# mengyao/Complete-Striped-Smith-Waterman-Library

Hardware: AMD Instinct MI355X
Metric: GCUPS (higher is better)
Workload: dtype int16x2 (packed; reference u8/int16 semantics); 1 GPU; BASELINE config 2: 100k x 150 bp reads vs 1 Mb target; 2/-2/3/1, score_size 2, flag 0; reads_per_gpu=100000, read_len=150, ref_len=1000000

## Files before the change

### complete-striped-smith-waterman-library_amd/csrc/lanes.h

```cpp
#ifndef SSW_LANES_H
#define SSW_LANES_H

#include <stdint.h>

typedef uint32_t u32;
typedef short s16x2 __attribute__((ext_vector_type(2)));
typedef unsigned short u16x2 __attribute__((ext_vector_type(2)));
typedef uint32_t u32x4 __attribute__((ext_vector_type(4)));
typedef uint32_t u32x2 __attribute__((ext_vector_type(2)));

#ifdef SSW_SIMT_EMU
#include "simt_emu.h"
#else
#include <hip/hip_runtime.h>
#define SSW_DEV __device__ __forceinline__
#define SSW_DEVM __device__ __forceinline__
#define SSW_HD __host__ __device__ inline
#define SSW_DYN_LDS(name) extern __shared__ __attribute__((aligned(16))) unsigned char name[]

SSW_DEV u32 xl_row_shr1_zero(u32 v) { return (u32)__builtin_amdgcn_mov_dpp((int)v, 0x111, 0xf, 0xf, true); }
SSW_DEV u32 xl_row_shr1_keep(u32 keep, u32 v) { return (u32)__builtin_amdgcn_update_dpp((int)keep, (int)v, 0x111, 0xf, 0xf, false); }
SSW_DEV u32 xl_row_shr1_umax(u32 v, u32 b)
{
	u32 r;
// ... 117 lines not shown
#define FR_DEAD 32768
SSW_DEV u32 fr_pack(int lo, int hi) { return (u32)lo + ((u32)hi << 16); }
SSW_DEV bool fr_borrows(u32 s0) { return (int32_t)s0 < 0 && s0 != fr_pack(FR_DEAD, FR_DEAD); }
template <bool HPAIR> SSW_DEV void fr_add_pair(u32 h0, u32 h1, u32 s0, u32 s1, u32& x0, u32& x1)
{
	unsigned long long h = (unsigned long long)h1 << 32 | h0, s = (unsigned long long)s1 << 32 | s0;
#ifdef SSW_SIMT_EMU
	if ((((unsigned long long)h0 + s0) >> 32 != 0) != fr_borrows(s0)) emu::fail("fr_add_pair: the low word's carry does not match its borrow");
#else
	asm("" : "+v"(s));
	if constexpr (HPAIR) asm("" : "+v"(h));
#endif
	const unsigned long long x = h + s;
	x0 = (u32)x; x1 = (u32)(x >> 32);
}
SSW_DEV u32 umax32(u32 a, u32 b) { return a > b ? a : b; }
#ifdef SSW_SIMT_EMU
SSW_DEV u32 pk_gt_mask(u32 a, u32 b) { return ((a & 0xffffu) > (b & 0xffffu) ? 0xffffu : 0u) | ((a >> 16) > (b >> 16) ? 0xffff0000u : 0u); }
#else
SSW_DEV u32 pk_gt_mask(u32 a, u32 b)
{
	u32 r;
	asm("v_pk_sub_u16 %0, %1, %2 clamp\n\tv_pk_min_u16 %0, %0, %3\n\tv_pk_mul_lo_u16 %0, %0, %4" : "=&v"(r) : "v"(a), "v"(b), "v"(0x00010001u), "v"(0xffffffffu));
	return r;
}
#endif
SSW_DEV u32 pk_addw(u32 a, u32 b) { return __builtin_bit_cast(u32, (u16x2)(__builtin_bit_cast(u16x2, a) + __builtin_bit_cast(u16x2, b))); }
SSW_DEV int fr_phi(int step, int lane, int GL, int base, int kmask, int gapE) { return base + ((step & kmask) + GL - lane) * gapE; }
SSW_DEV u32 pk_dup(int v) { return ((u32)v & 0xffffu) * 0x10001u; }
SSW_DEV u32 pk_make(int lo, int hi) { return ((u32)lo & 0xffffu) | ((u32)hi << 16); }
// ... 43 lines not shown
```

### complete-striped-smith-waterman-library_amd/csrc/ssw_dev.h

```cpp
#ifndef SSW_DEV_H
#define SSW_DEV_H

#include <stdint.h>
#include <stddef.h>

#ifdef __cplusplus
extern "C" {
#endif

#define SSW_RMAX 24
#define SSW_R8MAX 23
#define SSW_MAX_N 32
#define SSW_MAX_N_WIDE 128
#define SSW_LDS_LIMIT (160 * 1024)

typedef struct {
	int32_t qa;
	int32_t qb;
} ssw_pair;

typedef struct {
	int32_t score1, score2;
	int32_t ref_begin1, ref_end1, read_begin1, read_end1, ref_end2;
	int32_t cigarLen;
// ... 32 lines not shown
	const int8_t* mat;
	int32_t n;
	uint32_t gapO2, gapE2;
	int32_t tile;
	int32_t halo;
	int32_t ntiles;
	int32_t bpp;
	uint32_t* cm16;
	uint32_t* cm8;
	int64_t cm_stride;
	uint32_t* sg16;
	uint32_t* sg8;
	int64_t seg_stride;
	int32_t form;
	int32_t fr_base, fr_kmask;
} ssw_fill_args;

typedef struct {
	const ssw_fill_args* sub;
	const int32_t* first_wg;
	const int32_t* subR;
	int32_t nsub;
} ssw_fillm_args;

struct ssw_out_rec {
	uint16_t score1, score2;
	int32_t ref_begin1, ref_end1, read_begin1, read_end1, ref_end2, cigarLen, edit_distance;
	int64_t cigar_off;
	uint16_t flag, status;
};
// ... 454 lines not shown
```

### complete-striped-smith-waterman-library_amd/csrc/ssw_host.c

```c
#include <stdlib.h>
#include <stdio.h>
#include <string.h>
#include <pthread.h>
#include "ssw.h"
#include "ssw_gpu.h"
#ifdef SSW_GPU_TEST_HOOKS
#include "ssw_gpu_diag.h"
#endif
#include "ssw_dev.h"

_Static_assert(sizeof(struct ssw_out_rec) == sizeof(ssw_gpu_result), "device record layout must equal ssw_gpu_result");
_Static_assert(sizeof(struct ssw_mate_rec) == sizeof(ssw_gpu_mates) && sizeof(ssw_gpu_mates) == 32, "device selection layout must equal ssw_gpu_mates");
_Static_assert(sizeof(struct ssw_rescue_slot) == sizeof(ssw_gpu_rescued) && sizeof(ssw_gpu_rescued) == 24, "device rescue slot layout must equal ssw_gpu_rescued");
_Static_assert(SSW_MATES_GROUP_MAX == SSW_GPU_MATES_GROUP_MAX, "the kernel's group limit is the header's");
_Static_assert(SSW_MATES_FR == SSW_GPU_MATES_FR && SSW_MATES_RF == SSW_GPU_MATES_RF && SSW_MATES_FF == SSW_GPU_MATES_FF, "the kernel's orientations are the header's");
_Static_assert(sizeof(struct ssw_best_rec) == sizeof(ssw_gpu_best) && sizeof(ssw_gpu_best) == 16, "device record layout must equal ssw_gpu_best");

struct _profile {
	const int8_t* read;
	const int8_t* mat;
	int32_t readLen;
	int32_t n;
	int8_t score_size;
};
// ... 14 lines not shown
	int overlap;
	int no_track;
	int no_seg_reduce;
	int window_int16;
	int trace_wave;
	int trace_no_lds;
	int trace_waves;
	int trace_unblocked;
	int trace_many;
	int trace_early;
	int trace_w1max, trace_w4max, trace_headroom;
	int pipe_any_count;
	int pipe_low_prio;
	int pipe_parts;
	int no_fill_half;
	int no_pipe;
	int no_lit_spec;
	int trace_no_cls80;
	int trace_diag;
	int serial_buckets;
	int no_dbx;
	int no_tail;
	int no_band;
	int call_trace;
	int db_tsub, dbx_slab;
} ssw_knobs;

#define SSW_TSTREAMS 6
#define SSW_PSTREAMS 7
#define DB_STREAMS 4
// ... 21 lines not shown
	int budget_shrunk;
	ssw_knobs kn;
	int dev_cus, dev_wave_slots;
	int device_share;
	int queue_used;
	void* hits_d[2]; void* hits_h[2]; size_t hits_cap;
};

struct ssw_gpu_seqs {
	ssw_gpu_ctx* ctx;
	int8_t* d_codes;
	int64_t* d_off;
	int64_t* h_off;
	int32_t count;
	int64_t total;
};

static __thread char g_open_err[512];

#define CALL_TRACE(what) do { if (c->kn.call_trace) fprintf(stderr, "[ssw_gpu call] %9.3f ms  %s\n", dbg_ms(), what); } while (0)

#ifdef SSW_GPU_TEST_HOOKS
static int env_int(const char* name, int dflt) { const char* e = getenv(name); return e && e[0] ? atoi(e) : dflt; }
#endif
static int env_is(const char* name, char ch) { const char* e = getenv(name); return e && e[0] == ch; }
static void knobs_load(ssw_knobs* k)
{
	memset(k, 0, sizeof *k);
	k->debug = getenv("SSW_GPU_DEBUG") != 0;
	k->call_trace = env_is("SSW_GPU_CALL_TRACE", '1');
// ... 17 lines not shown
	k->no_seg_reduce = env_is("SSW_GPU_SEG_REDUCE", '0');
	k->window_int16 = getenv("SSW_GPU_WINDOW_INT16") != 0;
	k->trace_wave = getenv("SSW_GPU_TRACE_WAVE") ? env_is("SSW_GPU_TRACE_WAVE", '1') : -1;
	k->trace_no_lds = env_is("SSW_GPU_TRACE_LDS", '0');
	{ const int v = env_int("SSW_GPU_TRACE_WAVES", 0); k->trace_waves = v == 1 || v == 4 || v == 16 ? v : 0; }
	k->trace_unblocked = env_is("SSW_GPU_TRACE_BLOCKED", '0');
	k->trace_diag = env_is("SSW_GPU_TRACE_DIAG", '1');
	if (getenv("SSW_GPU_TRACE_MANY")) k->trace_many = env_int("SSW_GPU_TRACE_MANY", 4096);
	k->serial_buckets = env_is("SSW_GPU_SERIAL_BUCKETS", '1');
	k->no_dbx = env_is("SSW_GPU_NO_DBX", '1');
	k->no_band = env_is("SSW_GPU_NO_BAND", '1');
	k->trace_no_cls80 = env_is("SSW_GPU_TRACE_CLS80", '0');
	k->no_lit_spec = env_is("SSW_GPU_LIT_SPEC", '0');
	k->no_pipe = env_is("SSW_GPU_PIPE", '0');
	k->no_fill_half = env_is("SSW_GPU_FILL_HALF", '0');
	k->pipe_low_prio = env_is("SSW_GPU_PIPE_PRIO", 'l');
	k->pipe_any_count = env_is("SSW_GPU_PIPE_EVEN", '0');
	{ const int v = env_int("SSW_GPU_TRACE_W1MAX", 0); if (v >= 2 && v <= 254) k->trace_w1max = v; }
	{ const int v = env_int("SSW_GPU_TRACE_W4MAX", 0); if (v >= 2 && v <= 3070) k->trace_w4max = v; }
	{ const int v = env_int("SSW_GPU_TRACE_HEADROOM", 0); if (v >= 2 && v <= 64) k->trace_headroom = v; }
	{ const int v = env_int("SSW_GPU_PIPE_PARTS", 0); k->pipe_parts = v >= 2 && v <= 8 ? v : 0; }
	k->trace_early = env_int("SSW_GPU_TRACE_EARLY", 0);
	k->no_tail = env_is("SSW_GPU_NO_TAIL", '1');
	{ const int v = env_int("SSW_GPU_DB_TSUB", 0); k->db_tsub = v > 0 ? v : 0; }
	{ const int v = env_int("SSW_GPU_DBX_SLAB", 0); k->dbx_slab = v > 0 ? v : 0; }
#endif
}
#ifdef SSW_GPU_TEST_HOOKS
int ssw_gpu_has_test_hooks(void) { return 1; }
#endif
// ... 173 lines not shown
	return s;
}

ssw_gpu_seqs* ssw_gpu_seqs_upload(ssw_gpu_ctx* c, const int8_t* codes, const int64_t* offsets, int32_t count)
{
	if (!c || count < 0 || !offsets || (!codes && offsets[count] != offsets[0])) { fail(c, "seqs_upload: bad arguments%s", ""); return 0; }
	ssw_shim_set_device(c->device);
	ssw_gpu_seqs* s = seqs_new(c, offsets, count);
	if (!s) return 0;
	void* const us = upload_stream(c);
	if (ssw_shim_h2d(s->d_codes, codes + offsets[0], (size_t)s->total, us) ||
	    ssw_shim_h2d(s->d_off, s->h_off, sizeof(int64_t) * ((size_t)count + 1), us) ||
	    ssw_shim_stream_sync(us)) {
		fail(c, "upload failed: %s", ssw_shim_last_error()); ssw_gpu_seqs_free(s); return 0;
	}
	return s;
}

void ssw_gpu_seqs_free(ssw_gpu_seqs* s)
{
	if (!s) return;
	if (s->ctx) ssw_shim_set_device(s->ctx->device);
	ssw_shim_free(s->d_codes); ssw_shim_free(s->d_off); free(s->h_off); free(s);
}

ssw_gpu_seqs* ssw_gpu_seqs_upload_ascii(ssw_gpu_ctx* c, const char* text, const int64_t* offsets, int32_t count, const int8_t* table128)
{
	if (!c || count < 0 || !offsets || !table128 || (!text && offsets[count] != offsets[0])) { fail(c, "seqs_upload_ascii: bad arguments%s", ""); return 0; }
	ssw_shim_set_device(c->device);
	ssw_gpu_seqs* s = seqs_new(c, offsets, count);
	if (!s) return 0;
	void* const us = upload_stream(c);
	uint8_t* d_text = (uint8_t*)ssw_shim_malloc((size_t)s->total + 64);
	int8_t* d_tab = (int8_t*)ssw_shim_malloc(128);
	int ok = d_text && d_tab;
	if (ok) {
		ssw_prep_args pa; memset(&pa, 0, sizeof pa);
		pa.text = d_text; pa.table = d_tab; pa.off = s->d_off; pa.count = count; pa.total = s->total; pa.out = s->d_codes; pa.mode = 0;
		ok = !(ssw_shim_h2d(d_text, text + offsets[0], (size_t)s->total, us) || ssw_shim_h2d(d_tab, table128, 128, us) ||
		       ssw_shim_h2d(s->d_off, s->h_off, sizeof(int64_t) * ((size_t)count + 1), us) ||
		       ssw_shim_launch_prep(&pa, us) || ssw_shim_stream_sync(us));
	}
	ssw_shim_free(d_text); ssw_shim_free(d_tab);
	if (!ok) { fail(c, "ascii upload failed: %s", ssw_shim_last_error()); ssw_gpu_seqs_free(s); return 0; }
	return s;
}

ssw_gpu_seqs* ssw_gpu_seqs_revcomp(ssw_gpu_ctx* c, const ssw_gpu_seqs* in)
{
	if (!c || !in || in->ctx != c) { fail(c, "seqs_revcomp: bad arguments%s", ""); return 0; }
	ssw_shim_set_device(c->device);
	ssw_gpu_seqs* s = seqs_new(c, in->h_off, in->count);
	if (!s) return 0;
	void* const us = upload_stream(c);
	ssw_prep_args pa; memset(&pa, 0, sizeof pa);
	pa.codes_in = in->d_codes; pa.off = in->d_off; pa.count = in->count; pa.total = in->total; pa.out = s->d_codes; pa.mode = 1;
	if (ssw_shim_h2d(s->d_off, s->h_off, sizeof(int64_t) * ((size_t)in->count + 1), us) ||
	    ssw_shim_launch_prep(&pa, us) || ssw_shim_stream_sync(us)) {
		fail(c, "revcomp failed: %s", ssw_shim_last_error()); ssw_gpu_seqs_free(s); return 0;
	}
	return s;
}

ssw_gpu_seqs* ssw_gpu_seqs_with_revcomp(ssw_gpu_ctx* c, const ssw_gpu_seqs* in)
{
	if (!c || !in || in->ctx != c || in->count > 0x3fffffff) { fail(c, "seqs_with_revcomp: bad arguments%s", ""); return 0; }
	ssw_shim_set_device(c->device);
	const int32_t n = in->count;
	int64_t* off2 = (int64_t*)malloc(sizeof(int64_t) * (2 * (size_t)n + 1));
	if (!off2) { fail(c, "out of host memory%s", ""); return 0; }
	for (int32_t i = 0; i <= n; ++i) { off2[i] = in->h_off[i]; off2[n + i] = in->total + in->h_off[i]; }
	ssw_gpu_seqs* s = seqs_new(c, off2, 2 * n);
	free(off2);
	if (!s) return 0;
	void* const us = upload_stream(c);
	ssw_prep_args pa; memset(&pa, 0, sizeof pa);
	pa.codes_in = in->d_codes; pa.off = in->d_off; pa.count = n; pa.total = in->total; pa.out = s->d_codes; pa.mode = 2;
	if (ssw_shim_h2d(s->d_off, s->h_off, sizeof(int64_t) * (2 * (size_t)n + 1), us) ||
	    ssw_shim_launch_prep(&pa, us) || ssw_shim_stream_sync(us)) {
		fail(c, "revcomp failed: %s", ssw_shim_last_error()); ssw_gpu_seqs_free(s); return 0;
	}
	return s;
}

int ssw_gpu_seqs_download(ssw_gpu_ctx* c, const ssw_gpu_seqs* s, int8_t* codes_out)
{
	if (!c || !s || !codes_out) return -1;
	ssw_shim_set_device(c->device);
	if (ssw_shim_d2h(codes_out, s->d_codes, (size_t)s->total, c->stream) || ssw_shim_stream_sync(c->stream)) return fail(c, "download failed: %s", ssw_shim_last_error());
	return 0;
}

int32_t ssw_gpu_seqs_count(const ssw_gpu_seqs* s) { return s ? s->count : 0; }

int ssw_gpu_last_timing_sized(const ssw_gpu_ctx* c, void* out, size_t out_size)
{
// ... 5 lines not shown
int ssw_gpu_last_timing(const ssw_gpu_ctx* c, ssw_gpu_timing* out) { return ssw_gpu_last_timing_sized(c, out, sizeof *out); }


static int ssw_frame_params(const ssw_knobs* kn, int64_t top, int gapO, int gapE, int minmat, int lanes, int32_t* base, int32_t* kmask)
{
	if (gapO <= gapE || gapE < 1) return 0;
	int K = 1024;
	if (kn->frame_k) { K = 16; while (K * 2 <= kn->frame_k && K < 1024) K <<= 1; }
	while (K > 64 && (int64_t)K * gapE > 4096) K >>= 1;
	const int b = (minmat < 0 ? -minmat : 0) + gapO + 2 * gapE + 8;
	const int up = lanes + 2 + (lanes == 8 ? 3 : 0);
	while (K > 64 && top + b + (int64_t)(K + up) * gapE >= 31744) K >>= 1;
	if (top + b + (int64_t)(K + up) * gapE >= 31744) return 0;
	*base = b; *kmask = K - 1;
	return 1;
}

static int32_t halo_for(int32_t P, int32_t maxmat, int32_t gapE)
{
	if (gapE <= 0) return 0x3fffffff;
	int64_t w = (int64_t)P + ((int64_t)P * (maxmat > 0 ? maxmat : 0) + gapE - 1) / gapE + 1;
	return w > 0x3fffffff ? 0x3fffffff : (int32_t)w;
}

static void* next_event(ssw_gpu_ctx* c)
{
	if (c->nev == c->capev) {
		int nc = c->capev ? c->capev * 2 : 64;
		void** ne = (void**)realloc(c->ev, sizeof(void*) * nc);
		if (!ne) return 0;
// ... 166 lines not shown
typedef struct { int32_t key, need, q; } tpend;
static int tpend_cmp(const void* a, const void* b)
{
	const tpend* x = (const tpend*)a; const tpend* y = (const tpend*)b;
	if (x->key != y->key) return x->key < y->key ? -1 : 1;
	return x->q < y->q ? -1 : x->q > y->q;
}
static int keyed_cmp(const void* a, const void* b)
{
	const keyed* x = (const keyed*)a; const keyed* y = (const keyed*)b;
	if (x->key != y->key) return x->key < y->key ? -1 : 1;
	if (x->sub != y->sub) return x->sub < y->sub ? -1 : 1;
	return x->q < y->q ? -1 : (x->q > y->q);
}

static double fill8_ops_per_row(int R)
{
	if (R == 9) return 6.5;
	int cm = 0, last = 1;
	for (int k = 0; k < 4 && k < R; ++k) {
		const int n = (R - 1 - k) / 4 + 1 + (k == 0);
		cm += (n - 1) / 2;
		if (k == 0) last += (n & 1) == 0;
		else { cm += 1 + ((n & 1) == 0); ++last; }
	}
	return (double)(4 * R + (R + 1) / 2 + (R - 1) / 4 + cm + last / 2) / R;
}

static void note_fill_kernel(ssw_gpu_ctx* c, int64_t cells, int64_t* best_cells, const char* name, double ops, int32_t R, int32_t strips)
{
	if (cells <= *best_cells) return;
	*best_cells = cells;
	snprintf(c->tm.fill_kernel, sizeof c->tm.fill_kernel, "%s", name);
	c->tm.fill_ops_per_row = ops; c->tm.fill_rows_per_lane = R; c->tm.fill_strips = strips;
}

static int chainq_check(ssw_gpu_ctx* c)
{
	if (!c->queue_used || !c->qerr.p) return 0;
	int32_t e = 0;
	c->queue_used = 0;
// ... 1340 lines not shown
static int32_t* bucket_cand(const ssw_gpu_ctx* c, const target_plan* tp, const bucket* B, const bplan* P)
{
	return B->use_x && !c->kn.no_track ? (int32_t*)(tp->base_cand + P->cand_off) : 0;
}

static int fill_args_for(const ssw_gpu_ctx* c, const batch_call* bc, const target_plan* tp, const bucket* B, const bplan* P, int32_t p0, int32_t np,
                         const fill_bufs* fb, int half, ssw_fill_args* fa)
{
	const ssw_gpu_params* prm = bc->prm;
	const int64_t top = (int64_t)16 * B->R * (bc->maxmat > 0 ? bc->maxmat : 0);
	fa->tgt = tp->d_tgt; fa->refLen = tp->refLen; fa->qcodes = bc->Q->d_codes; fa->qoff = bc->Q->d_off;
	fa->pairs = bc->d_pairs + B->first_pair + p0; fa->npairs = np; fa->mat = bc->d_mat; fa->n = bc->n;
	fa->gapO2 = bc->gapO2; fa->gapE2 = bc->gapE2; fa->tile = P->tile; fa->halo = P->halo; fa->ntiles = P->ntiles;
	fa->bpp = (P->ntiles + 15) / 16; fa->cm16 = fb->cm16; fa->cm8 = fb->cm8; fa->cm_stride = tp->stride;
	fa->sg16 = fb->sg16; fa->sg8 = fb->sg8; fa->seg_stride = tp->seg_stride;
	fa->form = 0; fa->fr_base = 0; fa->fr_kmask = 0;
	if (bc->fill_form != 0 && ssw_frame_params(&c->kn, top, prm->gapO, prm->gapE, bc->minmat, 16, &fa->fr_base, &fa->fr_kmask)) fa->form = 3;
	int32_t hb = 0, hk = 0;
	if (!half || B->use_x || fa->form != 3 || !ssw_frame_params(&c->kn, top, prm->gapO, prm->gapE, bc->minmat, 8, &hb, &hk)) return 0;
	fa->fr_base = hb; fa->fr_kmask = hk;
	return 1;
}

static void reduce_args_for(const ssw_gpu_ctx* c, const batch_call* bc, const target_plan* tp, const bucket* B, const bplan* P, int32_t p0, int32_t np,
                            const fill_bufs* fb, ssw_reduce_args* ra)
{
	const ssw_gpu_params* prm = bc->prm;
	ra->cm16 = fb->cm16; ra->cm8 = fb->cm8; ra->cm_stride = tp->stride; ra->refLen = tp->refLen; ra->pairs = bc->d_pairs + B->first_pair + p0; ra->npairs = np;
	ra->qoff = bc->Q->d_off; ra->maskLen = prm->maskLen; ra->bias = bc->bias; ra->score_size = prm->score_size;
	ra->flag = prm->flag; ra->filters = prm->filters; ra->res = bc->d_res; ra->cand = bucket_cand(c, tp, B, P); ra->tile = P->tile; ra->ntiles = P->ntiles;
	ra->sg16 = fb->sg16; ra->sg8 = fb->sg8; ra->seg_stride = tp->seg_stride;
}

static int fill_launch(ssw_gpu_ctx* c, batch_call* bc, const target_plan* tp, int b, int32_t p0, int32_t np, const fill_bufs* fb, void* st, int* ndefer)
{
	const bucket* B = &bc->bk[b]; const bplan* P = &tp->bp[b];
	const ssw_gpu_params* prm = bc->prm;
	const int use_x = B->use_x, conc = ndefer != 0;
	const int32_t n = bc->n, refLen = tp->refLen, tile = P->tile, halo = P->halo, ntiles = P->ntiles;
	ssw_fill_args fa;
	const int use_half = fill_args_for(c, bc, tp, B, P, p0, np, fb, B->half && !conc, &fa);
	int xform = 0;
	if (use_x) {
		int32_t xfr_base = 0, xfr_kmask = 0;
		if (bc->fill_form != 0 && B->lanes == 64 &&
		    ssw_frame_params(&c->kn, (int64_t)B->P16 * (bc->maxmat > 0 ? bc->maxmat : 0), prm->gapO, prm->gapE, bc->minmat, 64, &xfr_base, &xfr_kmask)) xform = 3;
		ssw_chainx_args xa; memset(&xa, 0, sizeof xa);
		xa.tgt = tp->d_tgt; xa.refLen = refLen; xa.qcodes = bc->Q->d_codes; xa.qoff = bc->Q->d_off; xa.mat = bc->d_mat; xa.n = n;
		xa.gapO2 = bc->gapO2; xa.gapE2 = bc->gapE2; xa.gapE = prm->gapE; xa.maxmat = bc->maxmat; xa.njobs = np * ntiles;
		xa.pairs = fa.pairs; xa.tile = tile; xa.halo = halo; xa.ntiles = ntiles; xa.cm16 = fb->cm16; xa.cm8 = fb->cm8;
		xa.cm_stride = tp->stride; xa.bnd = (uint32_t*)(tp->base_bnd + P->bnd_off); xa.bnd_stride = P->maxcols; xa.cand = bucket_cand(c, tp, B, P); xa.lanes = B->lanes;
		xa.sg16 = fb->sg16; xa.sg8 = fb->sg8; xa.seg_stride = tp->seg_stride;
		if (B->lanes == 64) {
			const int qgrid = chainq_grid(c, B->R, 0, n);
			if (conc ? chainq_setup(c, &xa, B->strips, (int64_t)np * ntiles, qgrid, tp->base_q + P->q_off, tp->base_cs + P->cs_off, st)
			         : chainq_prepare(c, &xa, B->strips, (int64_t)np * ntiles, qgrid)) return -1;
// ... 8 lines not shown
	if (conc) {
		fill_defer* d = &bc->defer[(*ndefer)++];
		d->fa = fa; d->R = B->R; d->wgs = (int64_t)np * fa.bpp; d->group = ssw_shim_fill_class(B->R) * 2 + (fa.form == 3);
	} else
	if (use_half ? ssw_shim_launch_fill8(B->half, &fa, st) : ssw_shim_launch_fill(B->R, &fa, st)) return fail(c, "fill launch failed: %s", ssw_shim_last_error());

	int64_t cols = 0;
	for (int32_t k = 0; k < ntiles; ++k) {
		int64_t lo = (int64_t)k * tile, hi = lo + tile < refLen ? lo + tile : refLen;
		int64_t cf = lo - halo > 0 ? lo - halo : 0;
		cols += hi - cf;
	}
	const int64_t lc = cols * (int64_t)(use_half ? 8 * B->half : B->lanes * (B->tailR ? B->R * (B->strips - 1) + B->tailR : B->R * B->strips)) * 2 * np;
	c->tm.fill_cells += lc;
	char nm[48];
	if (use_half) snprintf(nm, sizeof nm, "k_fill8<%d,frame>", B->half);
	else if (!use_x) snprintf(nm, sizeof nm, "k_fill<%d,%s>", B->R, fa.form == 3 ? "frame" : "int16");
	else if (B->lanes == 64 && B->tailR) snprintf(nm, sizeof nm, "k_chainq<%d,%s> x %d strips + 1 of %d", B->R, xform == 3 ? "frame" : "int16", B->strips - 1, B->tailR);
	else if (B->lanes == 64) snprintf(nm, sizeof nm, "k_chainq<%d,%s> x %d strips", B->R, xform == 3 ? "frame" : "int16", B->strips);
	else snprintf(nm, sizeof nm, "k_chainx<%d,16 lanes> x %d strips", B->R, B->strips);
	note_fill_kernel(c, lc, &bc->best_fill_cells, nm, use_half ? fill8_ops_per_row(B->half) : !use_x ? (fa.form == 3 ? 6.5 : 9.0) : (B->lanes == 64 && xform == 3 ? 6.5 : 9.0), use_half ? B->half : B->R, B->strips);
	return 0;
}

static int fill_bucket_series(ssw_gpu_ctx* c, batch_call* bc, const target_plan* tp, int b)
{
	const bucket* B = &bc->bk[b]; const bplan* P = &tp->bp[b];
	const int dbl = P->dbl;
	const int pipe = P->pipe;
	const fill_bufs A = bucket_bufs(tp, P);
	fill_bufs B2 = A;
	if (dbl) { B2.cm16 = (uint32_t*)tp->base_cmB16; B2.cm8 = (uint32_t*)tp->base_cmB8; }
	void *pe0 = 0, *pe1 = 0;
	if (pipe) {
		pe0 = next_event(c); pe1 = next_event(c);
		if (ssw_shim_event_record(pe0, c->stream)) return fail(c, "stream wait failed: %s", ssw_shim_last_error());
// ... 1138 lines not shown
		free(q2); free(gidx); free(gbeg); free(goff); free(tmp);
		q2 = (int32_t*)malloc(sizeof(int32_t) * 2 * (size_t)m); t2 = q2 ? q2 + m : 0;
		gidx = (int32_t*)malloc(sizeof(int32_t) * (size_t)nd); gbeg = (int64_t*)malloc(sizeof(int64_t) * (size_t)nd);
		goff = (int64_t*)malloc(sizeof(int64_t) * ((size_t)nd + 1)); tmp = (ssw_gpu_result*)malloc(sizeof(ssw_gpu_result) * (size_t)m);
		if (!q2 || !gidx || !gbeg || !goff || !tmp) { fail(c, "out of host memory%s", ""); goto out; }
		int64_t d = -1;
		goff[0] = 0;
		for (int64_t k = k0; k < k1; ++k) {
			if (k == k0 || wk[k].t != wk[k - 1].t || wk[k].b != wk[k - 1].b || wk[k].l != wk[k - 1].l) {
				++d; gidx[d] = wk[k].t; gbeg[d] = wk[k].b; goff[d + 1] = goff[d] + wk[k].l;
			}
			q2[k - k0] = qidx[wk[k].i]; t2[k - k0] = (int32_t)d;
		}
		ssw_gpu_seqs* G = seqs_new(c, goff, (int32_t)nd);
		if (!G) goto out;
		unsigned char* d_g = (unsigned char*)ssw_shim_malloc(12 * (size_t)nd);
		ssw_seqgather_args ga; memset(&ga, 0, sizeof ga);
		ga.src = T->d_codes; ga.src_off = T->d_off; ga.src_beg = (const int64_t*)d_g; ga.idx = (const int32_t*)(d_g + 8 * (size_t)nd);
		ga.dst_off = G->d_off; ga.dst = G->d_codes; ga.count = (int32_t)nd;
		const int ok = d_g && !ssw_shim_h2d((void*)ga.src_beg, gbeg, 8 * (size_t)nd, c->stream) && !ssw_shim_h2d((void*)ga.idx, gidx, 4 * (size_t)nd, c->stream) &&
		               !ssw_shim_h2d(G->d_off, G->h_off, sizeof(int64_t) * ((size_t)nd + 1), c->stream) &&
		               !ssw_shim_launch_seqgather(&ga, c->stream) && !ssw_shim_stream_sync(c->stream);
		ssw_shim_free(d_g);
		if (!ok) { fail(c, "align_windows: window gather failed: %s", ssw_shim_last_error()); ssw_gpu_seqs_free(G); goto out; }
		uint32_t* pool = 0; int64_t words = 0;
		if (align_pairs_locked(c, Q, G, q2, t2, m, prm, tmp, &pool, &words)) { ssw_gpu_seqs_free(G); goto out; }
		ssw_gpu_seqs_free(G);
		timing_add(acc, &c->tm);
		acc->t.win_copied += sum;
		if (stage_append_batch(c, st, pool, words, tmp, m, &wk[k0].i, sizeof(wkey), results)) goto out;
// ... 821 lines not shown
```

### complete-striped-smith-waterman-library_amd/csrc/ssw_kernels.hip

```cpp
#include "lanes.h"
#include "ssw_dev.h"

#define DEAD2 0x80008000u

SSW_DEV int vm_query(const ssw_vmap& m, int v) { return m.vq ? m.vq[v] : v; }
SSW_DEV const int8_t* vm_target(const ssw_vmap& m, const int8_t* tgt, int v) { return m.vq ? m.tcodes + (m.win ? m.win[m.vt[v]].start : m.toff[m.vt[v]]) : tgt; }

#define RING_BYTES 160
#define CHAIN_BYTES (RING_BYTES + 256 + 256)

template <int R> struct ChainGeom {
	static constexpr int C = (R + 3) / 4;
	static constexpr int PSTRIDE = C * 256;
	static constexpr int A8 = 16 * R - 8;
	static constexpr int TAP = A8 / R;
	static constexpr int K8 = A8 % R;
};

template <int R, int PM = 0>
SSW_DEV void build_profile(unsigned char* lds, u32 base, int first, int nthreads,
                           const int8_t* mat, int n,
                           const int8_t* qa, int lena, int reva,
                           const int8_t* qb, int lenb, int p16a = 0x7fffffff, int p16b = 0x7fffffff, int gapE = 0)
{
// ... 252 lines not shown
template <int... I> struct RowSeq {};
template <int N, int... I> struct RowSeqTo : RowSeqTo<N - 1, N - 1, I...> {};
template <int... I> struct RowSeqTo<0, I...> { typedef RowSeq<I...> type; };
template <int R, int... I> SSW_DEV void rows_set(Rows8<R>& a, u32 v, RowSeq<I...>) { ((row_at<I>(a) = v), ...); }
template <int R, int... I> SSW_DEV void rows_sub(Rows8<R>& a, u32 k, RowSeq<I...>) { ((row_at<I>(a) -= k), ...); }

template <int R> struct RowFrame8 {
	static constexpr int P = R == 9 ? 1 : 4;
	static constexpr int cls(int r) { return r % P; }
	static constexpr int KL = cls(R - 1);
	static constexpr int count(int k) { return k < R && k < P ? (R - 1 - k) / P + 1 + (k == 0) : 0; }
	static constexpr bool LEFT0 = (count(0) & 1) == 0;
	static constexpr int ROW0 = (R - 1) / P * P;
	static constexpr bool PAIR = P != 1;
	static constexpr bool HPAIR = R <= 7;
};
template <int R, int... I> SSW_DEV void rows_set_cls(Rows8<R>& a, u32 v, u32 g, RowSeq<I...>) { ((row_at<I>(a) = v + (u32)RowFrame8<R>::cls(I) * g), ...); }
SSW_DEV u32 pk_max_all(u32 a) { return a; }
SSW_DEV u32 pk_max_all(u32 a, u32 b) { return pk_max(a, b); }
template <typename... T> SSW_DEV u32 pk_max_all(u32 a, u32 b, u32 c, T... rest) { return pk_max_all(pk_max3_fr(a, b, c), rest...); }

template <int R, int r>
SSW_DEV void chain_row8(const u32x4* sc, Rows8<R>& H, Rows8<R>& E, u32& x, u32& x2, u32& f, u32& a0, u32& a1, u32& a2, u32& a3,
                        u32 c1, u32 gapE2, u32 fl0, u32 fl1, u32 fl2, u32 fl3)
{
	typedef RowFrame8<R> F;
	constexpr int P = F::P, k = F::cls(r), j = r / P + (k == 0), n = F::count(k);
	u32& Hr = row_at<r>(H); u32& Er = row_at<r>(E);
	u32& a = k == 0 ? a0 : k == 1 ? a1 : k == 2 ? a2 : a3;
	u32 xn = 0u;
	if constexpr (F::PAIR && (r & 1) == 0) xn = x2;
	else if constexpr (F::PAIR && r + 2 < R) fr_add_pair<F::HPAIR>(Hr, row_at<(r + 2 < R ? r + 1 : 0)>(H), sc[(r + 1) >> 2][(r + 1) & 3], sc[(r + 1) >> 2][(r + 2) & 3], xn, x2);
	else if constexpr (r + 1 < R) xn = Hr + sc[(r + 1) >> 2][(r + 1) & 3];
	const u32 h = pk_max3_fr(x, Er, f);
	const u32 t = h - c1;
	Er = pk_max3_fr(Er, t, k == 0 ? fl0 : k == 1 ? fl1 : k == 2 ? fl2 : fl3);
	f = pk_max(f, t);
	if (r != R - 1 && F::cls(r + 1) == 0) f -= (u32)(k + 1) * gapE2;
	if (j == 0) a = h;
	else if ((j & 1) == 0) a = pk_max3_fr(a, row_at<(r >= P ? r - P : 0)>(H), h);
	else if (j == n - 1 && k != 0) a = pk_max(a, h);
	Hr = h;
	x = xn;
}
template <int R>
SSW_DEV u32 cm_finish8(Rows8<R>& H, u32 a0, u32 a1, u32 a2, u32 a3, u32 gapE2)
{
	typedef RowFrame8<R> F;
	if constexpr (F::P == 1) {
		if constexpr (F::LEFT0) return pk_max_all(a0, row_at<F::ROW0>(H));
		else return a0;
	} else if constexpr (R >= 4) {
		const u32 b1 = a1 - gapE2, b2 = a2 - 2u * gapE2, b3 = a3 - 3u * gapE2;
		if constexpr (F::LEFT0) return pk_max_all(a0, row_at<F::ROW0>(H), b1, b2, b3);
		else return pk_max_all(a0, b1, b2, b3);
	} else if constexpr (R == 3) return pk_max_all(a0, row_at<0>(H), a1 - gapE2, a2 - 2u * gapE2);
	else if constexpr (R == 2) return pk_max_all(a0, row_at<0>(H), a1 - gapE2);
	else return pk_max_all(a0, row_at<0>(H));
}
template <int R, int... I>
SSW_DEV u32 chain_rows_fr8(const u32x4* sc, Rows8<R>& H, Rows8<R>& E, u32 d, u32& f, u32 cm, u32 c1, u32 gapE2,
                           u32 fl0, u32 fl1, u32 fl2, u32 fl3, RowSeq<I...>)
{
	u32 x, x2 = 0, a0 = cm, a1 = 0, a2 = 0, a3 = 0;
	if constexpr (RowFrame8<R>::PAIR && R >= 2) fr_add_pair<RowFrame8<R>::HPAIR>(d, row_at<0>(H), sc[0][0], sc[0][1], x, x2);
	else x = d + sc[0][0];
	(chain_row8<R, I>(sc, H, E, x, x2, f, a0, a1, a2, a3, c1, gapE2, fl0, fl1, fl2, fl3), ...);
	return cm_finish8<R>(H, a0, a1, a2, a3, gapE2);
}

template <int R>
SSW_DEV void build_profile8(unsigned char* lds, int first, int nthreads, const int8_t* mat, int n,
                            const int8_t* const (&q)[4], const int (&len)[4], bool live1, int gapE)
{
	constexpr int C = ChainGeom<R>::C;
	const int total = (n + 1) * C * 64;
	for (int w = first; w < total; w += nthreads) {
		const int b = w / (C * 64), rem = w - b * (C * 64);
		const int c = rem >> 6, l = (rem & 63) >> 2, k = rem & 3;
		const int ch = l >> 3, r = c * 4 + k, row = (l & 7) * R + r;
		u32 v;
		if (b == n || (ch && !live1)) v = fr_pack(FR_DEAD, FR_DEAD);
// ... 63 lines not shown
		if (live1) { o16[cm_stride + tc] = i16[1]; o8[cm_stride + tc] = i8[1]; }
	}
	if (gq) {
		u32 m[4];
#pragma unroll
		for (int k = 0; k < 4; ++k) m[k] = in ? (k & 1 ? i8[k >> 1] : i16[k >> 1]) : 0u;
		const u32 x16 = pk_max(xl_dpp_banks<0x128, 0xc>(m[0], m[2]), xl_dpp_banks<0x128, 0x3>(m[2], m[0]));
		const u32 x8 = pk_max(xl_dpp_banks<0x128, 0xc>(m[1], m[3]), xl_dpp_banks<0x128, 0x3>(m[3], m[1]));
		u32 y = pk_max(xl_dpp_banks<0x114, 0xa>(x16, x8), xl_dpp_banks<0x104, 0x5>(x8, x16));
		y = pk_max(y, xl_dpp_banks<DPP_QUAD_SWAP1, 0xf>(y, y));
		y = pk_max(y, xl_dpp_banks<DPP_QUAD_SWAP2, 0xf>(y, y));
		if ((l16 & 3) == 0 && (live1 || l16 < 8) && base >= store_from && base < ncols) gq[base >> 4] = y;
	}
}

template <int R>
SSW_DEV void fill_body8(const ssw_fill_args& a, const int bid, unsigned char* lds)
{
	typedef ChainGeom<R> G;
	constexpr int C = G::C;
	const int tid = (int)threadIdx.x, l16 = tid & 15, grp = tid >> 4, ch = l16 & 1, pos = l16 >> 1;
	const int pg = bid / a.bpp, tchunk = bid - pg * a.bpp;
	const bool live1 = 2 * pg + 1 < a.npairs;
	const int gapEi = (int)(a.gapE2 & 0xffffu), gapOi = (int)(a.gapO2 & 0xffffu);
	const u32 prof_bytes = (u32)(a.n + 1) * G::PSTRIDE;
	const u32 ring = prof_bytes + (u32)grp * CHAIN8_BYTES;
	const u32 rb = opaque(ring + RING_BYTES), outv = rb + 2 * PARK8_BYTES + 2 * CRING8_BYTES, carry = outv + 2 * VRING8_BYTES;
	const u32 nulloff = (u32)a.n * G::PSTRIDE;

	{
		const int8_t* q[4]; int len[4];
#pragma unroll
		for (int k = 0; k < 2; ++k) {
// ... 38 lines not shown
		if (code < 0 || code > a.n) code = a.n;
		nxt = (u32)code * G::PSTRIDE;
	}
	__syncthreads();

	const u32 zero0 = pk_dup(fr_phi(0, pos, 8, a.fr_base, a.fr_kmask, gapEi) - gapEi);
	constexpr int KL = RowFrame8<R>::KL;
	const u32 klg = (u32)KL * a.gapE2;
	u32 fl0 = zero0 + a.gapE2, fl1 = fl0 + a.gapE2, fl2 = fl1 + a.gapE2, fl3 = fl2 + a.gapE2;
	typedef typename RowSeqTo<R>::type Rows;
	Rows8<R> H, E;
	rows_set_cls(H, zero0, a.gapE2, Rows()); rows_set_cls(E, fl0, a.gapE2, Rows());
	u32 Hlast = zero0 + klg, Fout = zero0 + klg + a.gapE2, cmout = zero0, hsave = zero0 + klg;
	const u32 lane_prof = (u32)(ch * 8 + pos) * 16u;
	const u32 gO = a.gapO2 - a.gapE2, gE = a.gapE2;
	const u32 gEv = opaque(klg + gE);
	u32 fin = 0;
	const u32 park = rb + (u32)ch * PARK8_BYTES, rbl = opaque(rb + 4u * (u32)l16);
	const u32 lgd = pk_dup(l16 * gapEi);
	const bool low8 = l16 < 8;

	for (int s0 = 0; s0 < nsteps; s0 += 16) {
		if (s0 > 0 && (s0 & a.fr_kmask) == 0) {
			const u32 k = (u32)(a.fr_kmask + 1) * a.gapE2;
			rows_sub(H, k, Rows()); rows_sub(E, k, Rows());
			Hlast -= k; Fout -= k; cmout -= k; hsave -= k; fl0 -= k; fl1 -= k; fl2 -= k; fl3 -= k;
		}
		{
			const int p = (s0 + 16 + l16) & 63;
			lds_st16(lds, ring + 2u * p, nxt);
// ... 9 lines not shown
		if (s0 >= 32)
			fill_flush8(lds, rb, s0 - 32, l16, store_from, ncols, live1, o16, o8, a.cm_stride, gq, gapEi, gapOi);
		const u32 rp = ring + 2u * (u32)((s0 - pos) & 63);
#pragma unroll
		for (int j = 0; j < 16; ++j) {
			const u32 paddr = lds_ld16(lds, rp + 2u * j) + lane_prof;
			u32x4 sc[C];
#pragma unroll
			for (int c = 0; c < C; ++c) sc[c] = lds_ld128(lds, paddr + 256u * c);
			const u32 hprev = Hlast;
			const u32 hin = xl_row_shr2_umax(Hlast, KL == 0 ? fl0 : KL == 1 ? fl1 : KL == 2 ? fl2 : fl3);
			if constexpr (RowFrame8<R>::P == 1) fl0 += gE;
			else { const u32 up = fl3 + gE; fl0 = fl1; fl1 = fl2; fl2 = fl3; fl3 = up; }
			xl_row_shr2_sub_keep(fin, Fout, gEv);
			u32 f = fin, d = hsave;
			const u32 cm = chain_rows_fr8(sc, H, E, d, f, xl_row_shr2_zero(cmout), gO, gE, fl0, fl1, fl2, fl3, Rows());
			hsave = hin; Hlast = row_at<R - 1>(H); Fout = f; cmout = cm;
			if (pos == 7) {
				lds_st32(lds, park + 4u * j, cm); lds_st32(lds, park + 64u + 4u * j, f); lds_st32(lds, park + 128u + 4u * j, hprev);
			}
		}
	}
	wave_lds_fence();
	fill_stage8(lds, rbl, nsteps - 16, low8, lgd, a.fr_base, a.fr_kmask, gapEi, gE, klg);
	wave_lds_fence();
	for (int base = nsteps - 32; base < nsteps; base += 16)
		if (base >= 0) fill_flush8(lds, rb, base, l16, store_from, ncols, live1, o16, o8, a.cm_stride, gq, gapEi, gapOi);
}

template <int R>
__global__ void __launch_bounds__(256) SSW_WAVES_PER_EU(R <= 9 ? 7 : R <= 15 ? 5 : 4, 8) k_fill8(ssw_fill_args a)
{
	SSW_DYN_LDS(lds);
	fill_body8<R>(a, (int)blockIdx.x, lds);
}

template <int CLS> struct FillClass { static constexpr int LO = CLS == 0 ? 1 : CLS == 1 ? 11 : 17, HI = CLS == 0 ? 10 : CLS == 1 ? 16 : 24; };
template <int R, int CLS, int FORM> SSW_DEV void fillm_case(const ssw_fill_args& a, int bid, unsigned char* lds)
{
	if (R >= FillClass<CLS>::LO && R <= FillClass<CLS>::HI) fill_body<(R >= FillClass<CLS>::LO && R <= FillClass<CLS>::HI) ? R : FillClass<CLS>::LO, FORM>(a, bid, lds);
}
template <int CLS, int FORM>
__global__ void __launch_bounds__(256) SSW_WAVES_PER_EU(CLS == 0 ? 7 : 1, 8) k_fillm(ssw_fillm_args m)
{
	SSW_DYN_LDS(lds);
	int s = 0;
	while (s + 1 < m.nsub && (int)blockIdx.x >= m.first_wg[s + 1]) ++s;
	const ssw_fill_args a = m.sub[s];
	const int bid = (int)blockIdx.x - m.first_wg[s];
// ... 3619 lines not shown
		FOR_EACH_R(X)
#undef X
		default: return -2;
	}
	return SSW_LAUNCH_OK();
}

extern "C" int ssw_shim_launch_fill8(int R8, const ssw_fill_args* a, void* stream)
{
	ssw_fill_args args = *a;
	const int64_t grid = (int64_t)((args.npairs + 1) / 2) * args.bpp;
	if (grid <= 0) return 0;
	if (args.form != 3) return -2;
	switch (R8) {
#define X(r) case r: { const size_t ldsb = (size_t)(args.n + 1) * ChainGeom<r>::PSTRIDE + 16 * CHAIN8_BYTES; \
		SSW_LAUNCH((k_fill8<r>), ssw_fill_args, args, grid, 256, ldsb, stream); } break;
		X(1) X(3) X(5) X(7) X(9) X(11) X(13) X(15) X(17) X(19) X(21) X(23)
#undef X
		default: return -2;
	}
	return SSW_LAUNCH_OK();
}

#define FOR_EACH_DBR_LONG(X) X(25) X(26) X(27) X(28) X(29) X(30) X(31) X(32) X(33) X(34) X(35) X(36) X(37) X(38) X(39) X(40)

extern "C" int ssw_shim_launch_filldb(int R, const ssw_filldb_args* a, void* stream)
{
	ssw_filldb_args args = *a;
	const int nch = SSW_DB_NCH;
	const int64_t grid = (int64_t)args.npairs * ((args.ntl + nch - 1) / nch);
	if (grid <= 0) return 0;
// ... 431 lines not shown
```

Baseline: 12570 GCUPS.

## Derive gap-open candidates from the diagonal sum in the 8-bit fill kernel

```diff
diff --git a/complete-striped-smith-waterman-library_amd/csrc/lanes.h b/complete-striped-smith-waterman-library_amd/csrc/lanes.h
--- a/complete-striped-smith-waterman-library_amd/csrc/lanes.h
+++ b/complete-striped-smith-waterman-library_amd/csrc/lanes.h
@@ -155,6 +155,28 @@
 	const unsigned long long x = h + s;
 	x0 = (u32)x; x1 = (u32)(x >> 32);
 }
+SSW_DEV void fr_sub_pair(u32& x0, u32& x1, u32 c, unsigned long long nc, u32& y0, u32& y1)
+{
+	unsigned long long x = (unsigned long long)x1 << 32 | x0;
+#ifdef SSW_SIMT_EMU
+	const u32 ch = c & 0xffffu;
+	if ((x0 & 0x7fffu) < ch || ((x0 >> 16) & 0x7fffu) < ch || (x1 & 0x7fffu) < ch || ((x1 >> 16) & 0x7fffu) < ch || x0 < c)
+		emu::fail("fr_sub_pair: a borrow crosses a half or a word");
+	if (x + nc != ((unsigned long long)(x1 - c) << 32 | (x0 - c))) emu::fail("fr_sub_pair: the pair subtract differs from the two 32-bit subtracts");
+#else
+	asm("" : "+v"(x));
+	x0 = (u32)x; x1 = (u32)(x >> 32);
+#endif
+	const unsigned long long y = x + nc;
+	y0 = (u32)y; y1 = (u32)(y >> 32);
+}
+SSW_DEV u32 fr_sub_one(u32 x, u32 c)
+{
+#ifdef SSW_SIMT_EMU
+	if ((x & 0x7fffu) < (c & 0xffffu) || ((x >> 16) & 0x7fffu) < (c & 0xffffu)) emu::fail("fr_sub_one: a borrow crosses a half");
+#endif
+	return x - c;
+}
 SSW_DEV u32 umax32(u32 a, u32 b) { return a > b ? a : b; }
 #ifdef SSW_SIMT_EMU
 SSW_DEV u32 pk_gt_mask(u32 a, u32 b) { return ((a & 0xffffu) > (b & 0xffffu) ? 0xffffu : 0u) | ((a >> 16) > (b >> 16) ? 0xffff0000u : 0u); }
diff --git a/complete-striped-smith-waterman-library_amd/csrc/ssw_dev.h b/complete-striped-smith-waterman-library_amd/csrc/ssw_dev.h
--- a/complete-striped-smith-waterman-library_amd/csrc/ssw_dev.h
+++ b/complete-striped-smith-waterman-library_amd/csrc/ssw_dev.h
@@ -70,6 +70,7 @@
 	int64_t seg_stride;
 	int32_t form;
 	int32_t fr_base, fr_kmask;
+	int32_t dg;
 } ssw_fill_args;
 
 typedef struct {
diff --git a/complete-striped-smith-waterman-library_amd/csrc/ssw_host.c b/complete-striped-smith-waterman-library_amd/csrc/ssw_host.c
--- a/complete-striped-smith-waterman-library_amd/csrc/ssw_host.c
+++ b/complete-striped-smith-waterman-library_amd/csrc/ssw_host.c
@@ -52,6 +52,7 @@
 	int pipe_low_prio;
 	int pipe_parts;
 	int no_fill_half;
+	int no_fill_dg;
 	int no_pipe;
 	int no_lit_spec;
 	int trace_no_cls80;
@@ -103,6 +104,7 @@
 	int64_t* h_off;
 	int32_t count;
 	int64_t total;
+	int codes_ranged; int32_t code_lo, code_hi;
 };
 
 static __thread char g_open_err[512];
@@ -150,6 +152,7 @@
 	k->no_lit_spec = env_is("SSW_GPU_LIT_SPEC", '0');
 	k->no_pipe = env_is("SSW_GPU_PIPE", '0');
 	k->no_fill_half = env_is("SSW_GPU_FILL_HALF", '0');
+	k->no_fill_dg = env_is("SSW_GPU_FILL_DG", '0');
 	k->pipe_low_prio = env_is("SSW_GPU_PIPE_PRIO", 'l');
 	k->pipe_any_count = env_is("SSW_GPU_PIPE_EVEN", '0');
 	{ const int v = env_int("SSW_GPU_TRACE_W1MAX", 0); if (v >= 2 && v <= 254) k->trace_w1max = v; }
@@ -353,6 +356,12 @@
 	    ssw_shim_stream_sync(us)) {
 		fail(c, "upload failed: %s", ssw_shim_last_error()); ssw_gpu_seqs_free(s); return 0;
 	}
+	{
+		const int8_t* p = codes + offsets[0];
+		int lo = 127, hi = -128;
+		for (int64_t i = 0; i < s->total; ++i) { if (p[i] < lo) lo = p[i]; if (p[i] > hi) hi = p[i]; }
+		s->codes_ranged = 1; s->code_lo = lo; s->code_hi = hi;
+	}
 	return s;
 }
 
@@ -382,7 +391,16 @@
 	}
 	ssw_shim_free(d_text); ssw_shim_free(d_tab);
 	if (!ok) { fail(c, "ascii upload failed: %s", ssw_shim_last_error()); ssw_gpu_seqs_free(s); return 0; }
+	s->codes_ranged = 1; s->code_lo = 127; s->code_hi = -128;
+	for (int i = 0; i < 128; ++i) { if (table128[i] < s->code_lo) s->code_lo = table128[i]; if (table128[i] > s->code_hi) s->code_hi = table128[i]; }
 	return s;
+}
+
+static void seqs_range_revcomp(ssw_gpu_seqs* s, const ssw_gpu_seqs* in)
+{
+	s->codes_ranged = in->codes_ranged;
+	s->code_lo = in->code_lo < 0 || in->code_lo > in->code_hi ? in->code_lo : 0;
+	s->code_hi = in->code_hi > 3 || in->code_lo > in->code_hi ? in->code_hi : 3;
 }
 
 ssw_gpu_seqs* ssw_gpu_seqs_revcomp(ssw_gpu_ctx* c, const ssw_gpu_seqs* in)
@@ -398,6 +416,7 @@
 	    ssw_shim_launch_prep(&pa, us) || ssw_shim_stream_sync(us)) {
 		fail(c, "revcomp failed: %s", ssw_shim_last_error()); ssw_gpu_seqs_free(s); return 0;
 	}
+	seqs_range_revcomp(s, in);
 	return s;
 }
 
@@ -419,6 +438,7 @@
 	    ssw_shim_launch_prep(&pa, us) || ssw_shim_stream_sync(us)) {
 		fail(c, "revcomp failed: %s", ssw_shim_last_error()); ssw_gpu_seqs_free(s); return 0;
 	}
+	seqs_range_revcomp(s, in);
 	return s;
 }
 
@@ -454,6 +474,13 @@
 	if (top + b + (int64_t)(K + up) * gapE >= 31744) return 0;
 	*base = b; *kmask = K - 1;
 	return 1;
+}
+
+static int fill8_diag_gaps(const ssw_knobs* kn, const ssw_gpu_seqs* T, int R8, int32_t n, int32_t minmat, int gapO, int gapE)
+{
+	if (kn->no_fill_dg || R8 == 9 || R8 == 17 || gapO <= gapE) return 0;
+	if (-(int64_t)minmat > 2 * (int64_t)gapE) return 0;
+	return T->codes_ranged && (T->code_lo > T->code_hi || (T->code_lo >= 0 && T->code_hi < n));
 }
 
 static int32_t halo_for(int32_t P, int32_t maxmat, int32_t gapE)
@@ -650,7 +677,7 @@
 	return x->q < y->q ? -1 : (x->q > y->q);
 }
 
-static double fill8_ops_per_row(int R)
+static double fill8_ops_per_row(int R, int dg)
 {
 	if (R == 9) return 6.5;
 	int cm = 0, last = 1;
@@ -660,7 +687,8 @@
 		if (k == 0) last += (n & 1) == 0;
 		else { cm += 1 + ((n & 1) == 0); ++last; }
 	}
-	return (double)(4 * R + (R + 1) / 2 + (R - 1) / 4 + cm + last / 2) / R;
+	const double ops = (double)((dg ? 3 : 4) * R + (dg ? 2 : 1) * ((R + 1) / 2) + (R - 1) / 4 + cm + last / 2) / R;
+	return dg && ops < 5.0 ? 5.0 : ops;
 }
 
 static void note_fill_kernel(ssw_gpu_ctx* c, int64_t cells, int64_t* best_cells, const char* name, double ops, int32_t R, int32_t strips)
@@ -2031,11 +2059,12 @@
 	fa->gapO2 = bc->gapO2; fa->gapE2 = bc->gapE2; fa->tile = P->tile; fa->halo = P->halo; fa->ntiles = P->ntiles;
 	fa->bpp = (P->ntiles + 15) / 16; fa->cm16 = fb->cm16; fa->cm8 = fb->cm8; fa->cm_stride = tp->stride;
 	fa->sg16 = fb->sg16; fa->sg8 = fb->sg8; fa->seg_stride = tp->seg_stride;
-	fa->form = 0; fa->fr_base = 0; fa->fr_kmask = 0;
+	fa->form = 0; fa->fr_base = 0; fa->fr_kmask = 0; fa->dg = 0;
 	if (bc->fill_form != 0 && ssw_frame_params(&c->kn, top, prm->gapO, prm->gapE, bc->minmat, 16, &fa->fr_base, &fa->fr_kmask)) fa->form = 3;
 	int32_t hb = 0, hk = 0;
 	if (!half || B->use_x || fa->form != 3 || !ssw_frame_params(&c->kn, top, prm->gapO, prm->gapE, bc->minmat, 8, &hb, &hk)) return 0;
 	fa->fr_base = hb; fa->fr_kmask = hk;
+	fa->dg = fill8_diag_gaps(&c->kn, bc->T, half, bc->n, bc->minmat, prm->gapO, prm->gapE);
 	return 1;
 }
 
@@ -2056,7 +2085,7 @@
 	const int use_x = B->use_x, conc = ndefer != 0;
 	const int32_t n = bc->n, refLen = tp->refLen, tile = P->tile, halo = P->halo, ntiles = P->ntiles;
 	ssw_fill_args fa;
-	const int use_half = fill_args_for(c, bc, tp, B, P, p0, np, fb, B->half && !conc, &fa);
+	const int use_half = fill_args_for(c, bc, tp, B, P, p0, np, fb, B->half && !conc ? B->half : 0, &fa);
 	int xform = 0;
 	if (use_x) {
 		int32_t xfr_base = 0, xfr_kmask = 0;
@@ -2095,12 +2124,12 @@
 	const int64_t lc = cols * (int64_t)(use_half ? 8 * B->half : B->lanes * (B->tailR ? B->R * (B->strips - 1) + B->tailR : B->R * B->strips)) * 2 * np;
 	c->tm.fill_cells += lc;
 	char nm[48];
-	if (use_half) snprintf(nm, sizeof nm, "k_fill8<%d,frame>", B->half);
+	if (use_half) snprintf(nm, sizeof nm, fa.dg ? "k_fill8<%d,frame> dg" : "k_fill8<%d,frame>", B->half);
 	else if (!use_x) snprintf(nm, sizeof nm, "k_fill<%d,%s>", B->R, fa.form == 3 ? "frame" : "int16");
 	else if (B->lanes == 64 && B->tailR) snprintf(nm, sizeof nm, "k_chainq<%d,%s> x %d strips + 1 of %d", B->R, xform == 3 ? "frame" : "int16", B->strips - 1, B->tailR);
 	else if (B->lanes == 64) snprintf(nm, sizeof nm, "k_chainq<%d,%s> x %d strips", B->R, xform == 3 ? "frame" : "int16", B->strips);
 	else snprintf(nm, sizeof nm, "k_chainx<%d,16 lanes> x %d strips", B->R, B->strips);
-	note_fill_kernel(c, lc, &bc->best_fill_cells, nm, use_half ? fill8_ops_per_row(B->half) : !use_x ? (fa.form == 3 ? 6.5 : 9.0) : (B->lanes == 64 && xform == 3 ? 6.5 : 9.0), use_half ? B->half : B->R, B->strips);
+	note_fill_kernel(c, lc, &bc->best_fill_cells, nm, use_half ? fill8_ops_per_row(B->half, fa.dg) : !use_x ? (fa.form == 3 ? 6.5 : 9.0) : (B->lanes == 64 && xform == 3 ? 6.5 : 9.0), use_half ? B->half : B->R, B->strips);
 	return 0;
 }
 
@@ -3269,6 +3298,7 @@
 		}
 		ssw_gpu_seqs* G = seqs_new(c, goff, (int32_t)nd);
 		if (!G) goto out;
+		G->codes_ranged = T->codes_ranged; G->code_lo = T->code_lo; G->code_hi = T->code_hi;
 		unsigned char* d_g = (unsigned char*)ssw_shim_malloc(12 * (size_t)nd);
 		ssw_seqgather_args ga; memset(&ga, 0, sizeof ga);
 		ga.src = T->d_codes; ga.src_off = T->d_off; ga.src_beg = (const int64_t*)d_g; ga.idx = (const int32_t*)(d_g + 8 * (size_t)nd);
diff --git a/complete-striped-smith-waterman-library_amd/csrc/ssw_kernels.hip b/complete-striped-smith-waterman-library_amd/csrc/ssw_kernels.hip
--- a/complete-striped-smith-waterman-library_amd/csrc/ssw_kernels.hip
+++ b/complete-striped-smith-waterman-library_amd/csrc/ssw_kernels.hip
@@ -290,34 +290,46 @@
 	static constexpr int ROW0 = (R - 1) / P * P;
 	static constexpr bool PAIR = P != 1;
 	static constexpr bool HPAIR = R <= 7;
+	static constexpr bool DG = PAIR && R != 17;
 };
 template <int R, int... I> SSW_DEV void rows_set_cls(Rows8<R>& a, u32 v, u32 g, RowSeq<I...>) { ((row_at<I>(a) = v + (u32)RowFrame8<R>::cls(I) * g), ...); }
 SSW_DEV u32 pk_max_all(u32 a) { return a; }
 SSW_DEV u32 pk_max_all(u32 a, u32 b) { return pk_max(a, b); }
 template <typename... T> SSW_DEV u32 pk_max_all(u32 a, u32 b, u32 c, T... rest) { return pk_max_all(pk_max3_fr(a, b, c), rest...); }
 
-template <int R, int r>
-SSW_DEV void chain_row8(const u32x4* sc, Rows8<R>& H, Rows8<R>& E, u32& x, u32& x2, u32& f, u32& a0, u32& a1, u32& a2, u32& a3,
-                        u32 c1, u32 gapE2, u32 fl0, u32 fl1, u32 fl2, u32 fl3)
+template <int R, int r, bool DG>
+SSW_DEV void chain_row8(const u32x4* sc, Rows8<R>& H, Rows8<R>& E, u32& x, u32& x2, u32& xc, u32& xc2, u32& f, u32& a0, u32& a1, u32& a2, u32& a3,
+                        u32 c1, unsigned long long nc1, u32 gapE2, u32 fl0, u32 fl1, u32 fl2, u32 fl3)
 {
 	typedef RowFrame8<R> F;
 	constexpr int P = F::P, k = F::cls(r), j = r / P + (k == 0), n = F::count(k);
 	u32& Hr = row_at<r>(H); u32& Er = row_at<r>(E);
 	u32& a = k == 0 ? a0 : k == 1 ? a1 : k == 2 ? a2 : a3;
-	u32 xn = 0u;
-	if constexpr (F::PAIR && (r & 1) == 0) xn = x2;
-	else if constexpr (F::PAIR && r + 2 < R) fr_add_pair<F::HPAIR>(Hr, row_at<(r + 2 < R ? r + 1 : 0)>(H), sc[(r + 1) >> 2][(r + 1) & 3], sc[(r + 1) >> 2][(r + 2) & 3], xn, x2);
-	else if constexpr (r + 1 < R) xn = Hr + sc[(r + 1) >> 2][(r + 1) & 3];
+	u32 xn = 0u, xcn = 0u;
+	if constexpr (F::PAIR && (r & 1) == 0) { xn = x2; xcn = xc2; }
+	else if constexpr (F::PAIR && r + 2 < R) {
+		fr_add_pair<F::HPAIR>(Hr, row_at<(r + 2 < R ? r + 1 : 0)>(H), sc[(r + 1) >> 2][(r + 1) & 3], sc[(r + 1) >> 2][(r + 2) & 3], xn, x2);
+		if constexpr (DG) fr_sub_pair(xn, x2, c1, nc1, xcn, xc2);
+	} else if constexpr (r + 1 < R) {
+		xn = Hr + sc[(r + 1) >> 2][(r + 1) & 3];
+		if constexpr (DG) xcn = fr_sub_one(xn, c1);
+	}
 	const u32 h = pk_max3_fr(x, Er, f);
-	const u32 t = h - c1;
-	Er = pk_max3_fr(Er, t, k == 0 ? fl0 : k == 1 ? fl1 : k == 2 ? fl2 : fl3);
-	f = pk_max(f, t);
+	if constexpr (DG) {
+		const u32 fl = k == 0 ? fl0 : k == 1 ? fl1 : k == 2 ? fl2 : fl3;
+		Er = pk_max3_fr(xc, Er, fl);
+		f = pk_max3_fr(xc, f, fl);
+	} else {
+		const u32 t = h - c1;
+		Er = pk_max3_fr(Er, t, k == 0 ? fl0 : k == 1 ? fl1 : k == 2 ? fl2 : fl3);
+		f = pk_max(f, t);
+	}
 	if (r != R - 1 && F::cls(r + 1) == 0) f -= (u32)(k + 1) * gapE2;
 	if (j == 0) a = h;
 	else if ((j & 1) == 0) a = pk_max3_fr(a, row_at<(r >= P ? r - P : 0)>(H), h);
 	else if (j == n - 1 && k != 0) a = pk_max(a, h);
 	Hr = h;
-	x = xn;
+	x = xn; xc = xcn;
 }
 template <int R>
 SSW_DEV u32 cm_finish8(Rows8<R>& H, u32 a0, u32 a1, u32 a2, u32 a3, u32 gapE2)
@@ -334,14 +346,19 @@
 	else if constexpr (R == 2) return pk_max_all(a0, row_at<0>(H), a1 - gapE2);
 	else return pk_max_all(a0, row_at<0>(H));
 }
-template <int R, int... I>
-SSW_DEV u32 chain_rows_fr8(const u32x4* sc, Rows8<R>& H, Rows8<R>& E, u32 d, u32& f, u32 cm, u32 c1, u32 gapE2,
+template <bool DG, int R, int... I>
+SSW_DEV u32 chain_rows_fr8(const u32x4* sc, Rows8<R>& H, Rows8<R>& E, u32 d, u32& f, u32 cm, u32 c1, unsigned long long nc1, u32 gapE2,
                            u32 fl0, u32 fl1, u32 fl2, u32 fl3, RowSeq<I...>)
 {
-	u32 x, x2 = 0, a0 = cm, a1 = 0, a2 = 0, a3 = 0;
-	if constexpr (RowFrame8<R>::PAIR && R >= 2) fr_add_pair<RowFrame8<R>::HPAIR>(d, row_at<0>(H), sc[0][0], sc[0][1], x, x2);
-	else x = d + sc[0][0];
-	(chain_row8<R, I>(sc, H, E, x, x2, f, a0, a1, a2, a3, c1, gapE2, fl0, fl1, fl2, fl3), ...);
+	u32 x, x2 = 0, xc = 0, xc2 = 0, a0 = cm, a1 = 0, a2 = 0, a3 = 0;
+	if constexpr (RowFrame8<R>::PAIR && R >= 2) {
+		fr_add_pair<RowFrame8<R>::HPAIR>(d, row_at<0>(H), sc[0][0], sc[0][1], x, x2);
+		if constexpr (DG) fr_sub_pair(x, x2, c1, nc1, xc, xc2);
+	} else {
+		x = d + sc[0][0];
+		if constexpr (DG) xc = fr_sub_one(x, c1);
+	}
+	(chain_row8<R, I, DG>(sc, H, E, x, x2, xc, xc2, f, a0, a1, a2, a3, c1, nc1, gapE2, fl0, fl1, fl2, fl3), ...);
 	return cm_finish8<R>(H, a0, a1, a2, a3, gapE2);
 }
 
@@ -435,9 +452,10 @@
 	}
 }
 
-template <int R>
+template <int R, bool DG>
 SSW_DEV void fill_body8(const ssw_fill_args& a, const int bid, unsigned char* lds)
 {
+	static_assert(!DG || RowFrame8<R>::DG, "gaps from the diagonal: no such instance");
 	typedef ChainGeom<R> G;
 	constexpr int C = G::C;
 	const int tid = (int)threadIdx.x, l16 = tid & 15, grp = tid >> 4, ch = l16 & 1, pos = l16 >> 1;
@@ -506,6 +524,7 @@
 	u32 Hlast = zero0 + klg, Fout = zero0 + klg + a.gapE2, cmout = zero0, hsave = zero0 + klg;
 	const u32 lane_prof = (u32)(ch * 8 + pos) * 16u;
 	const u32 gO = a.gapO2 - a.gapE2, gE = a.gapE2;
+	const unsigned long long ngO = 0ull - ((unsigned long long)gO << 32 | gO);
 	const u32 gEv = opaque(klg + gE);
 	u32 fin = 0;
 	const u32 park = rb + (u32)ch * PARK8_BYTES, rbl = opaque(rb + 4u * (u32)l16);
@@ -545,7 +564,7 @@
 			else { const u32 up = fl3 + gE; fl0 = fl1; fl1 = fl2; fl2 = fl3; fl3 = up; }
 			xl_row_shr2_sub_keep(fin, Fout, gEv);
 			u32 f = fin, d = hsave;
-			const u32 cm = chain_rows_fr8(sc, H, E, d, f, xl_row_shr2_zero(cmout), gO, gE, fl0, fl1, fl2, fl3, Rows());
+			const u32 cm = chain_rows_fr8<DG>(sc, H, E, d, f, xl_row_shr2_zero(cmout), gO, ngO, gE, fl0, fl1, fl2, fl3, Rows());
 			hsave = hin; Hlast = row_at<R - 1>(H); Fout = f; cmout = cm;
 			if (pos == 7) {
 				lds_st32(lds, park + 4u * j, cm); lds_st32(lds, park + 64u + 4u * j, f); lds_st32(lds, park + 128u + 4u * j, hprev);
@@ -559,11 +578,11 @@
 		if (base >= 0) fill_flush8(lds, rb, base, l16, store_from, ncols, live1, o16, o8, a.cm_stride, gq, gapEi, gapOi);
 }
 
-template <int R>
+template <int R, bool DG>
 __global__ void __launch_bounds__(256) SSW_WAVES_PER_EU(R <= 9 ? 7 : R <= 15 ? 5 : 4, 8) k_fill8(ssw_fill_args a)
 {
 	SSW_DYN_LDS(lds);
-	fill_body8<R>(a, (int)blockIdx.x, lds);
+	fill_body8<R, DG>(a, (int)blockIdx.x, lds);
 }
 
 template <int CLS> struct FillClass { static constexpr int LO = CLS == 0 ? 1 : CLS == 1 ? 11 : 17, HI = CLS == 0 ? 10 : CLS == 1 ? 16 : 24; };
@@ -4213,7 +4232,9 @@
 	if (args.form != 3) return -2;
 	switch (R8) {
 #define X(r) case r: { const size_t ldsb = (size_t)(args.n + 1) * ChainGeom<r>::PSTRIDE + 16 * CHAIN8_BYTES; \
-		SSW_LAUNCH((k_fill8<r>), ssw_fill_args, args, grid, 256, ldsb, stream); } break;
+		if (args.dg && !RowFrame8<r>::DG) return -2; \
+		if (args.dg) SSW_LAUNCH((k_fill8<r, RowFrame8<r>::DG>), ssw_fill_args, args, grid, 256, ldsb, stream); \
+		else SSW_LAUNCH((k_fill8<r, false>), ssw_fill_args, args, grid, 256, ldsb, stream); } break;
 		X(1) X(3) X(5) X(7) X(9) X(11) X(13) X(15) X(17) X(19) X(21) X(23)
 #undef X
 		default: return -2;
```

Result: faster. 13510 GCUPS (median of 6 runs) (+7.5%).
